# Rita-zi/WavTokenizer

Measured on AMD Instinct MI355X. Metric: audio-seconds/sec encode+decode, 24 kHz 3 s clips, higher is better.
Workload: dtype f32 (split-f16 x3 products)

## Files before the change

include/wavtokenizer_amd.h:

```cpp
#ifndef WAVTOKENIZER_AMD_H
#define WAVTOKENIZER_AMD_H

#include <stddef.h>
#include <stdint.h>

#ifdef __cplusplus
extern "C" {
#endif

typedef enum {
    WT_OK = 0,
    WT_ERR_INVALID = -1,
    WT_ERR_MISSING_TENSOR = -2,
    WT_ERR_SHAPE = -3,
    WT_ERR_HIP = -4,
    WT_ERR_NOT_INITED = -5,
    WT_ERR_RANGE = -6,
    WT_ERR_LSTM_SYNC = -7,
    WT_ERR_INDEX = -8
} wt_status;

enum wt_status_bits {
    WT_STATUS_BIT_LSTM = 1,
    WT_STATUS_BIT_RANGE = 2
// ... 140 lines not shown
    const float* B;
    const float* bias;
    const float* R;
    const float* gamma;
    float* C;
    float* C2;
    uint32_t* status;
} wt_gemm_desc;
typedef struct {
    int32_t BM, BN, waves_m, waves_n, stages, ks, prod, staged, bias_cache, G, tiles;
} wt_launch_form;
size_t wt_gemm_probe_workspace_bytes(const wt_gemm_desc* d);
int wt_gemm_probe(const wt_gemm_desc* d, wt_launch_form* form, void* workspace, void* stream);

enum { WT_OP_GN_APPLY = 0, WT_OP_GN_STATS = 1, WT_OP_ROWNORM = 2, WT_OP_SOFTMAX = 3, WT_OP_ISTFT_OLA = 4, WT_OP_CONV_FIRST = 5,
       WT_OP_CONV_LAST = 6, WT_OP_TRANSPOSE = 7, WT_OP_CONVTR = 8, WT_OP_ROW_SUMSQ = 9, WT_OP_S32_AMAX = 10 };
enum { WT_OPK_GN_TILE = 1, WT_OPK_GN_CHUNK = 2, WT_OPK_GN_STATS = 3, WT_OPK_ROWNORM = 4, WT_OPK_DWCONV_LN = 5,
       WT_OPK_SOFTMAX_REG = 6, WT_OPK_SOFTMAX_RMW = 7, WT_OPK_ISTFT_OLA = 8, WT_OPK_CONV_FIRST = 9, WT_OPK_CONV_LAST32 = 10,
       WT_OPK_CONV_LAST = 11, WT_OPK_TRANSPOSE = 12, WT_OPK_CONVTR = 13, WT_OPK_ROW_SUMSQ = 14, WT_OPK_S32_AMAX = 15 };
typedef struct {
    int32_t size;
    int32_t op;
    int32_t B, L, C;
    int32_t groups, mode, flag, out_s32;
    int32_t ld, k, stride, Cout, n_fft, hop, Kq;
    float eps;
    int64_t n;
    const void* x;
    const void *p0, *p1, *p2, *p3, *p4, *p5;
    void *y, *y2, *y3;
    uint32_t* status;
} wt_op_desc;
typedef struct {
    int32_t kernel;
    int32_t variant;
    int32_t variant2;
    int32_t grid_x, grid_y, grid_z, block, lds;
} wt_op_form;
int wt_op_probe(const wt_op_desc* d, wt_op_form* form, void* stream);

int wt_resblock(const float* x, const float* wav, const float* e0_w, const float* e0_b, const float* w3, const float* b3,
                const float* w1, const float* b1, const float* ws, const float* bs, float* y, int32_t B, int64_t T,
                int32_t C, int32_t elu_out, int32_t out_s32, int32_t fp32_chain, void* stream);
int wt_resblock_down(const float* wav, const float* e0_w, const float* e0_b, const float* w3, const float* b3, const float* w1,
                     const float* b1, const float* ws, const float* bs, const float* wd, const float* bd, float* y_down,
                     int32_t B, int64_t T, int32_t r, void* stream);

int wt_unit_run(const wt_plan* p, const float* x, float* y, void* workspace, void* stream);

int wt_model_take_bad_codes(const wt_model* m);


typedef struct wt_resampler wt_resampler;
int     wt_resampler_create(int32_t orig_sr, int32_t new_sr, int32_t device, wt_resampler** out);
void    wt_resampler_destroy(wt_resampler* r);
// ... 13 lines not shown
```

wavtokenizer_amd/_capi.py:

```python
from __future__ import annotations

import ctypes
import os
from ctypes import POINTER, c_char_p, c_float, c_int32, c_int64, c_size_t, c_void_p

_HERE = os.path.dirname(os.path.abspath(__file__))
LIB_PATH = os.environ.get("WAVTOK_HIP_LIB") or os.path.join(_HERE, "libwavtok_hip.so")

EXPORTS = [
    "wt_last_error", "wt_version", "wt_model_create", "wt_model_destroy", "wt_model_export_bytes", "wt_model_export", "wt_packed_info", "wt_packed_verify", "wt_packed_bytes",
    "wt_model_create_packed", "wt_model_hop", "wt_model_weight_bytes",
    "wt_plan_create", "wt_plan_create_ex", "wt_plan_range_sites", "wt_plan_range_report", "wt_model_persistent_lstm", "wt_device_info", "wt_plan_destroy", "wt_plan_workspace_bytes", "wt_plan_frames", "wt_plan_num_launches", "wt_plan_graph_replays",
    "wt_plan_find_buffer", "wt_plan_buffer_info", "wt_plan_buffer_name", "wt_plan_status", "wt_plan_num_steps", "wt_plan_step_name",
    "wt_plan_set_timing", "wt_plan_read_timing", "wt_model_split_ok", "wt_model_status", "wt_model_take_bad_codes", "wt_encode", "wt_codes_to_features",
    "wt_decode", "wt_seanet_decode", "wt_head", "wt_unit_run", "wt_sconv1d", "wt_linear", "wt_conv1d_s32", "wt_vq_workspace_bytes",
    "wt_vq_nearest", "wt_vq_nearest_f32", "wt_resblock", "wt_resblock_down", "wt_gemm_probe_workspace_bytes", "wt_gemm_probe", "wt_op_probe",
    "wt_resampler_create", "wt_resampler_destroy", "wt_resampler_out_length", "wt_convert_audio", "wt_pcm16",
    "wt_linear_overlap_add", "wt_encode_mixed", "wt_plan_min_clip_length", "wt_sconv_geometry",
]

WT_PLAN_ENCODE, WT_PLAN_DECODE, WT_PLAN_SEANET_DECODER, WT_PLAN_HEAD, WT_PLAN_UNIT_LSTM = 0, 1, 2, 3, 4
WT_PLAN_FLAG_KEEP_STAGES = 1
WT_PLAN_FLAG_FP32_GEMM = 2
WT_PLAN_FLAG_STEP_LSTM = 4
WT_PLAN_FLAG_GRAPH = 8
WT_PLAN_FLAG_UNFUSED = 16
WT_PLAN_FLAG_RANGE_REPORT = 32
WT_PLAN_FLAG_MIXED_LENGTH = 64
WT_SITE_ENCODER, WT_SITE_BB_EMBED, WT_SITE_RES0, WT_SITE_RES1, WT_SITE_ATTN, WT_SITE_RES2, WT_SITE_RES3 = 0, 1, 2, 3, 4, 5, 6
WT_SITE_CNX0, WT_SITE_HEAD, WT_SITE_SEANET_DECODER = 7, 40, 41
WT_ERR_INVALID = -1
# ... 18 lines not shown
                 ("M", c_int32), ("N", c_int32), ("K", c_int32)]
                + [(n, c_int32) for n in ("T_in", "T_out", "Cin", "taps", "stride", "dil", "pad_left", "pad_mode", "Tp",
                                         "K1", "nz", "tap_pair", "head_kb")]
                + [("alpha", c_float)]
                + [(n, c_int64) for n in ("a_bstride", "a_rstride", "a2_bstride", "a2_rstride", "w_rstride", "c_rstride",
                                         "r_rstride", "zA", "zW", "zC")]
                + [(n, c_void_p) for n in ("A", "A2", "B", "bias", "R", "gamma", "C", "C2", "status")])


class WtLaunchForm(ctypes.Structure):
    _fields_ = [(n, c_int32) for n in ("BM", "BN", "waves_m", "waves_n", "stages", "ks", "prod", "staged", "bias_cache", "G", "tiles")]


WT_OP_GN_APPLY, WT_OP_GN_STATS, WT_OP_ROWNORM, WT_OP_SOFTMAX, WT_OP_ISTFT_OLA, WT_OP_CONV_FIRST = 0, 1, 2, 3, 4, 5
WT_OP_CONV_LAST, WT_OP_TRANSPOSE, WT_OP_CONVTR, WT_OP_ROW_SUMSQ, WT_OP_S32_AMAX = 6, 7, 8, 9, 10
WT_OPK_NAMES = {1: "gn_tile", 2: "gn_chunk", 3: "gn_stats", 4: "rownorm", 5: "dwconv_ln", 6: "softmax_reg", 7: "softmax_rmw",
                8: "istft_ola", 9: "conv_first", 10: "conv_last32", 11: "conv_last", 12: "transpose", 13: "convtr",
                14: "row_sumsq", 15: "s32_amax"}


class WtOpDesc(ctypes.Structure):
    _fields_ = ([(n, c_int32) for n in ("size", "op", "B", "L", "C", "groups", "mode", "flag", "out_s32", "ld", "k", "stride",
                                        "Cout", "n_fft", "hop", "Kq")]
                + [("eps", c_float), ("n", c_int64)]
                + [(n, c_void_p) for n in ("x", "p0", "p1", "p2", "p3", "p4", "p5", "y", "y2", "y3", "status")])


class WtOpForm(ctypes.Structure):
    _fields_ = [(n, c_int32) for n in ("kernel", "variant", "variant2", "grid_x", "grid_y", "grid_z", "block", "lds")]


class WavTokError(RuntimeError):
    def __init__(self, msg, status=0):
# ... 74 lines not shown
    lib.wt_sconv1d.argtypes = [c_void_p, c_void_p, c_void_p, c_void_p, c_int32, c_int64, c_int32, c_int32, c_int32,
                               c_int32, c_int32, c_int32, c_void_p]
    lib.wt_linear.argtypes = [c_void_p, c_void_p, c_void_p, c_void_p, c_int64, c_int32, c_int32, c_int32, c_void_p, c_void_p]
    lib.wt_conv1d_s32.argtypes = [c_void_p, c_void_p, c_void_p, c_void_p, c_int32, c_int64, c_int32, c_int32, c_int32,
                                  c_int32, c_int32, c_void_p, c_void_p]
    lib.wt_vq_workspace_bytes.argtypes = [c_int64, c_int32, c_int32]
    lib.wt_vq_workspace_bytes.restype = c_size_t
    lib.wt_vq_nearest.argtypes = [c_void_p, c_void_p, c_int64, c_int32, c_int32, c_void_p, c_void_p, c_void_p]
    lib.wt_vq_nearest_f32.argtypes = [c_void_p, c_void_p, c_int64, c_int32, c_int32, c_void_p, c_void_p, c_void_p]
    lib.wt_resblock.argtypes = [c_void_p] * 11 + [c_int32, c_int64, c_int32, c_int32, c_int32, c_int32, c_void_p]
    lib.wt_resblock_down.argtypes = [c_void_p] * 12 + [c_int32, c_int64, c_int32, c_void_p]
    lib.wt_gemm_probe_workspace_bytes.argtypes = [POINTER(WtGemmDesc)]
    lib.wt_gemm_probe_workspace_bytes.restype = c_size_t
    lib.wt_gemm_probe.argtypes = [POINTER(WtGemmDesc), POINTER(WtLaunchForm), c_void_p, c_void_p]
    lib.wt_op_probe.argtypes = [POINTER(WtOpDesc), POINTER(WtOpForm), c_void_p]
    lib.wt_resampler_create.argtypes = [c_int32, c_int32, c_int32, POINTER(c_void_p)]
    lib.wt_resampler_destroy.argtypes = [c_void_p]
    lib.wt_resampler_destroy.restype = None
    lib.wt_resampler_out_length.argtypes = [c_void_p, c_int64]
    lib.wt_resampler_out_length.restype = c_int64
    lib.wt_convert_audio.argtypes = [c_void_p, c_void_p, c_int32, c_int32, c_int64, c_void_p, c_void_p]
    lib.wt_pcm16.argtypes = [c_void_p, c_int64, ctypes.c_float, c_int32, c_void_p, c_void_p, c_void_p]
    lib.wt_linear_overlap_add.argtypes = [c_void_p, c_void_p, c_int32, c_int64, c_int64, c_int64, c_int64, c_void_p, c_void_p]
    return lib


lib = _load()


def check(rc: int, what: str = "") -> None:
# ... 4 lines not shown
```

wavtokenizer_amd/csrc/capi.cpp:

```cpp
#include "model.h"

namespace wt {
static thread_local std::string g_err;
void set_error(const std::string& msg) { g_err = msg; }
thread_local LaunchCtx g_launch;
int device_cus() {
    static std::atomic<int> cache[64];
    int d = 0;
    (void)hipGetDevice(&d);
    d &= 63;
    int v = cache[d].load(std::memory_order_relaxed);
    if (v <= 0) {
        if (hipDeviceGetAttribute(&v, hipDeviceAttributeMultiprocessorCount, d) != hipSuccess || v <= 0) v = 256;
        cache[d].store(v, std::memory_order_relaxed);
    }
    return v;
}
}

using namespace wt;

static int alloc_host_words(wt_model* M, const char* who) {
    void* hp = nullptr;
    void* dp = nullptr;
// ... 728 lines not shown
            if (int rc = launch_fill_u32(scale_dev, bits, 16, s)) return rc;
            a.acc_scale = 1.f / scale;
        }
        if (int rc = launch_split_s32(d->B, ws + L.oB, L.nB, s, scale != 1.f ? scale_dev : nullptr)) return rc;
        if (int rc = launch_split_s32(d->A, ws, L.nA, s)) return rc;
        if (d->A2) if (int rc = launch_split_s32(d->A2, ws + L.oA2, L.nA2, s)) return rc;
        if (int rc = launch_gemm16s(a, d->epi, d->out, s)) return rc;
    }
    if (form) *form = wt_launch_form{lf.BM, lf.BN, lf.waves_m, lf.waves_n, lf.stages, lf.ks, lf.prod, lf.staged, lf.bias_cache, lf.G, lf.tiles};
    return WT_OK;
}

static int op_probe_check(const wt_op_desc* d) {
    auto bad = [](const char* m) { set_error(std::string("wt_op_probe: ") + m); return (int)WT_ERR_INVALID; };
    if (!d || d->size != (int32_t)sizeof(wt_op_desc)) return bad("descriptor missing or of another size");
    if (d->op < WT_OP_GN_APPLY || d->op > WT_OP_S32_AMAX) return bad("unknown op");
    auto al16 = [](const void* p) { return !(reinterpret_cast<uintptr_t>(p) & 15); };
    const void* ptrs[] = {d->p0, d->p1, d->p2, d->p3, d->p4, d->p5, d->y, d->y2, d->y3};
    for (const void* p : ptrs) if (!al16(p)) return bad("arrays must be 16-byte aligned");
    if (!d->x || (reinterpret_cast<uintptr_t>(d->x) & (d->op == WT_OP_SOFTMAX ? 3 : 15))) return bad("x missing or misaligned");
    if (reinterpret_cast<uintptr_t>(d->status) & 3) return bad("status misaligned");
    const bool shaped = d->op != WT_OP_SOFTMAX && d->op != WT_OP_ROW_SUMSQ && d->op != WT_OP_S32_AMAX;
    if (shaped && (d->B <= 0 || d->L <= 0)) return bad("extents must be positive");
    if (shaped && d->op != WT_OP_CONV_FIRST && d->op != WT_OP_ISTFT_OLA && (d->C <= 0 || (long)d->L * d->C >= (long)INT_MAX)) return bad("extents must be positive (and L * C < 2^31)");
    switch (d->op) {
    case WT_OP_GN_APPLY: case WT_OP_GN_STATS:
        if (!d->p0 || !d->p1 || !d->y2 || !d->y3 || (d->op == WT_OP_GN_APPLY && !d->y)) return bad("null argument");
        if (d->groups <= 0 || d->C % d->groups || d->C / d->groups > 256 || d->B > 65535) return bad("GroupNorm needs C % groups == 0, at most 256 channels per group, B <= 65535");
        break;
    case WT_OP_ROWNORM:
        if (!d->y || !d->p4 || !d->p5) return bad("null argument");
// ... 21 lines not shown
        if (!d->y) return bad("null argument");
        if (d->B > 65535 || (d->L + 31) / 32 > 65535) return bad("transpose: too many tiles for one launch");
        break;
    case WT_OP_CONVTR:
        if (!d->p0 || !d->p1 || !d->y) return bad("null argument");
        if (d->stride <= 0 || d->k < d->stride || d->Cout <= 0 || d->Cout % 4) return bad("convtr needs k >= stride > 0 and Cout % 4 == 0");
        break;
    case WT_OP_ROW_SUMSQ:
        if (!d->y) return bad("null argument");
        if (d->n <= 0 || d->C <= 0 || d->C % 4) return bad("row_sumsq needs rows > 0 and C % 4 == 0");
        break;
    case WT_OP_S32_AMAX:
        if (!d->y) return bad("null argument");
        if (d->n <= 0 || d->n % 32) return bad("s32_amax needs whole S32 groups of 32 values");
        break;
    }
    return WT_OK;
}

int wt_op_probe(const wt_op_desc* d, wt_op_form* form, void* stream) {
    if (int rc = op_probe_check(d)) return rc;
    hipStream_t s = static_cast<hipStream_t>(stream);
    auto F = [](const void* p) { return static_cast<const float*>(p); };
    auto W = [](void* p) { return static_cast<float*>(p); };
    OpForm lf;
    const LaunchCtx saved = g_launch;
    g_launch.status = reinterpret_cast<unsigned*>(d->status);
    g_launch.form = &lf;
    int rc = 0;
    switch (d->op) {
    case WT_OP_GN_APPLY:
        rc = launch_gn_apply(F(d->x), F(d->p0), F(d->p1), W(d->y2), W(d->y3), W(d->y), d->flag ? 1 : 0, d->B, d->L, d->C, d->groups, d->eps, s,
// ... 18 lines not shown
    case WT_OP_CONV_LAST:
        rc = launch_conv_last(F(d->x), F(d->p0), F(d->p1), W(d->y), d->B, d->L, d->C, d->k, d->flag ? 1 : 0, s);
        break;
    case WT_OP_TRANSPOSE:
        rc = launch_transpose(F(d->x), W(d->y), d->B, d->L, d->C, s, d->out_s32 ? 1 : 0);
        break;
    case WT_OP_CONVTR:
        rc = launch_convtr(F(d->x), F(d->p0), F(d->p1), W(d->y), d->B, d->L, d->C, d->Cout, d->k, d->stride, d->flag ? 1 : 0, s);
        break;
    case WT_OP_ROW_SUMSQ:
        rc = launch_row_sumsq(F(d->x), W(d->y), d->n, d->C, s);
        break;
    case WT_OP_S32_AMAX:
        rc = launch_s32_amax(d->x, d->n, static_cast<unsigned*>(d->y), s);
        break;
    }
    g_launch = saved;
    if (rc) return rc;
    if (form) *form = wt_op_form{lf.kernel, lf.variant, lf.variant2, (int32_t)lf.grid[0], (int32_t)lf.grid[1], (int32_t)lf.grid[2], (int32_t)lf.block, (int32_t)lf.lds};
    return WT_OK;
}

size_t wt_vq_workspace_bytes(int64_t N, int32_t D, int32_t bins) {
    const size_t np = std::max(gemm_vq_parts(bins), gemm16s_vq_parts(bins));
    return al256((size_t)N * D * 4) + al256((size_t)bins * D * 4) + al256((size_t)N * sizeof(float)) +
           2 * al256((size_t)N * np * sizeof(float)) + al256((size_t)bins * sizeof(float)) + 512;
}

static int vq_nearest(const float* x, const float* embed, int64_t N, int32_t D, int32_t bins, int64_t* codes_out,
                      void* workspace, void* stream, bool s32) {
// ... 69 lines not shown
```

wavtokenizer_amd/csrc/common.h:

```cpp
#pragma once
#include <hip/hip_runtime.h>
#include <stdint.h>
#include <stdio.h>
#include <stdlib.h>
#include <mutex>
#include <string>

namespace wt {

void set_error(const std::string& msg);

#define WT_HIP_CHECK(expr)                                                                      \
    do {                                                                                        \
        hipError_t _e = (expr);                                                                 \
        if (_e != hipSuccess) {                                                                 \
            ::wt::set_error(std::string(#expr) + ": " + hipGetErrorString(_e));                 \
            return -4;                                                                          \
        }                                                                                       \
    } while (0)

struct PerDeviceOnce {
    std::mutex mu;
    bool seen[64] = {};
    template <class F> int run(F&& f) {
        int d = 0;
        (void)hipGetDevice(&d);
        d &= 63;
        std::lock_guard<std::mutex> g(mu);
        if (seen[d]) return 0;
        if (int rc = f()) return rc;
        seen[d] = true;
        return 0;
    }
};

enum : unsigned { WT_STATUS_LSTM = 1u, WT_STATUS_RANGE = 2u };
enum OpKernel : int {
    OPK_NONE = 0, OPK_GN_TILE, OPK_GN_CHUNK, OPK_GN_STATS, OPK_ROWNORM, OPK_DWCONV_LN, OPK_SOFTMAX_REG, OPK_SOFTMAX_RMW,
    OPK_ISTFT_OLA, OPK_CONV_FIRST, OPK_CONV_LAST32, OPK_CONV_LAST, OPK_TRANSPOSE, OPK_CONVTR, OPK_ROW_SUMSQ, OPK_S32_AMAX
};
struct OpForm {
    int kernel = OPK_NONE;
    int variant = 0;
    int variant2 = 0;
    unsigned grid[3] = {0, 0, 0};
    unsigned block = 0;
    unsigned lds = 0;
};
struct LaunchCtx {
    unsigned* status = nullptr;
    OpForm* form = nullptr;
    unsigned long long* stamp_start = nullptr;
    unsigned long long* stamp_end = nullptr;
    bool stamp_used = false;
// ... 248 lines not shown
    int R;
};
struct ResblockMix {
    const int* T = nullptr;
    const int* Tread = nullptr;
};
bool resblock_fusable(int C);
int launch_resblock(const ResblockArgs& a, hipStream_t s);
int launch_resblock16(const ResblockArgs& a, hipStream_t s, const ResblockMix* mix = nullptr);
bool resblock16_down_fusable(int C, long T, int r, int k);
int launch_resblock16_down(const ResblockArgs& a, hipStream_t s, const ResblockMix* mix = nullptr);
int launch_mixed_geometry(const int* lengths, int* geom, int B, long Tpad, int tmin, int n_st, const int* kd, const int* rd,
                          int kf, hipStream_t s);
int launch_mixed_pad(const int* geom, int l_word, int64_t* codes, float* feat_ncl, float* emb_ncl, int B, int L, int D,
                     hipStream_t s);
int launch_convtr(const float* x, const float* w , const float* bias, float* y, int B, int Tin,
                  int Cin, int Cout, int k, int stride, int elu_in, hipStream_t s);

}
```

wavtokenizer_amd/csrc/model.h:

```cpp
#pragma once
#include "../../include/wavtokenizer_amd.h"
#include "common.h"

#include <algorithm>
#include <atomic>
#include <climits>
#include <cmath>
#include <cstring>
#include <functional>
#include <map>
#include <memory>
#include <mutex>
#include <string>
#include <vector>

namespace wt {

struct S32Copy {
    const void* p = nullptr;
    float acc_scale = 1.f;
    bool tap_pair = false;
};
struct ConvW {
    float* w = nullptr;
// ... 260 lines not shown

int build_model(wt_model* M, TensorMap& tm);
int build_splits(wt_model* M);
float s32_weight_scale(float amax);
size_t model_export_bytes(const wt_model* M);
int model_export(const wt_model* M, void* buf, size_t n);
int model_import(wt_model* M, const void* buf, size_t n);
int packed_info(const void* buf, size_t n, wt_arch* arch, int32_t* version, uint64_t* arch_hash);
int ensure_f32_weights(const wt_model* M);
size_t packed_bytes(const void* buf, size_t n);
int packed_verify(const void* buf, size_t n);
GemmArgs sconv_args(const ConvW& w, int B, long T, int stride, int dil);
GemmArgs zconv_args(const ConvW& w, int B, int L);
GemmArgs linear_args(const float* W, const float* bias, long M, int N, int K);
GemmArgs linear_args(const GemmW& W, const float* bias, long M, int N, int K);
int build_encode(wt_plan* P);
int build_decode(wt_plan* P);
int build_head(wt_plan* P);
int build_seanet_decoder(wt_plan* P);
int build_unit_lstm(wt_plan* P);
void plan_begin(wt_plan* P);
void plan_end(wt_plan* P);
inline long wave_samples(const wt_model* M, long L) {
    return M->arch.padding_same ? L * (long)M->arch.hop_length : (L - 1) * (long)M->arch.hop_length;
}

}
```

wavtokenizer_amd/csrc/plan.cpp:

```cpp
#include "model.h"

namespace wt {

static bool site_fp32(const wt_plan* P, int site) { return (P->fp32_sites >> site) & 1u; }
static bool plan_fp32(const wt_plan* P) {
    if ((P->flags & WT_PLAN_FLAG_FP32_GEMM) || !P->model->s32_ok) return true;
    if (P->kind == WT_PLAN_SEANET_DECODER) return !P->model->sd_s32_ok || site_fp32(P, SITE_SEADEC);
    if (P->kind == WT_PLAN_ENCODE || P->kind == WT_PLAN_UNIT_LSTM) return site_fp32(P, SITE_ENC);
    if (P->kind == WT_PLAN_HEAD) return site_fp32(P, SITE_HEAD);
    return false;
}
static bool plan_unfused(const wt_plan* P) { return P->flags & WT_PLAN_FLAG_UNFUSED; }
static bool plan_s32(const wt_plan* P) { return !plan_unfused(P) && !plan_fp32(P); }

static int gemm_auto(const wt_plan* P, const GemmArgs& a, int pro, int epi, hipStream_t s) {
    if (P->model->f32_stale.load()) if (int rc = ensure_f32_weights(P->model)) return rc;
    return launch_gemm(a, pro, epi, s);
}

static void set_s32(GemmArgs& a, const S32Copy& c) {
    a.W_hi = c.p; a.acc_scale = c.acc_scale; a.tap_pair = c.tap_pair ? 1 : 0;
}

static int gemm_s32(const GemmArgs& a, int epi, int out, hipStream_t s, const int* mix = nullptr) {
// ... 154 lines not shown
    });
    const int o = P->buf(name, (size_t)B * T * C, BUF_S32 | BUF_ELU);
    GemmArgs ac = sconv_args(sc, B, T, 1, 1);
    ac.W = cat.w; ac.w_rstride = cat.cin; ac.bias = cat.b; ac.K = cat.cin; ac.Cin = cat.cin;
    set_s32(ac, cat.s32);
    ac.K1 = C; ac.a2_bstride = T * (C / 2); ac.a2_rstride = C / 2;
    P->step({geom, x_raw, h, o}, [=](const RunCtx& c) {
        GemmArgs a = ac; a.A = P->ptr(c, x_raw) + x_off; a.A2 = P->ptr(c, h); a.C = P->ptr(c, o);
        if (x_bstride) a.a_bstride = x_bstride;
        const int* mix = geom >= 0 ? reinterpret_cast<const int*>(P->ptr(c, geom)) + mix_word + GEOM_SC : nullptr;
        return gemm_s32(a, EPI_BIAS_ELU, OUT_S32, c.stream, mix);
    });
    return o;
}

int build_encode(wt_plan* P) {
    const wt_model* M = P->model;
    const int B = P->B;
    const long T = P->T;
    const bool fold_e0 = !plan_unfused(P) && !M->stages.empty() && M->stages[0].C == 32 &&
                         M->e0_k == 7 && resblock_fusable(32);
    int x = -1;
    if (!fold_e0) {
        x = P->buf("enc.0", (size_t)B * T * M->e0_c);
        const int x0 = x;
        P->step({x0}, [=](const RunCtx& c) {
            return launch_conv_first(c.in_f, M->e0_w, M->e0_b, P->ptr(c, x0), B, T, M->e0_k, M->e0_c, c.stream);
        });
    }
    const bool fuse_elu = !plan_unfused(P);
    const bool s32 = plan_s32(P);
    struct Route { bool fused, down, s32; };
    std::vector<Route> route(M->stages.size());
    for (size_t si = 0; si < route.size(); ++si) {
        const ResStage& st = M->stages[si];
        Route& r = route[si];
        r.fused = resblock_fusable(st.C) && !plan_unfused(P);
        r.s32 = s32 && st.C % 32 == 0 && st.down.s32.p &&
                (r.fused || (si > 0 && route[si - 1].s32 && st.c3.s32.p && st.c1.s32.p && st.sc.s32.p));
        r.down = si == 0 && fold_e0 && r.fused && r.s32 && route.size() > 1 && resblock_fusable(M->stages[1].C) &&
                 st.down.cin == 32 && st.down.cout == 64 && resblock16_down_fusable(st.C, T, st.r, st.down.k);
    }
    const bool lstm_s32 = !route.empty() && route.back().s32 && M->enc_lstm.Wih0.s32.p;
    const bool tail_s32 = lstm_s32 && M->enc_final.s32.p && M->embed.s32.p;
    const bool mixed = P->flags & WT_PLAN_FLAG_MIXED_LENGTH;
    const int n_st = (int)route.size();
    int geom = -1;
    if (mixed) {
        bool ok = s32 && !(P->flags & (WT_PLAN_FLAG_KEEP_STAGES | WT_PLAN_FLAG_RANGE_REPORT)) && tail_s32 &&
                  n_st >= 2 && n_st <= GEOM_MAX_STAGES && route[0].down;
        for (int si = 1; si < n_st && ok; ++si)
            ok = route[si].s32 && (route[si].fused ? M->stages[si].C == 64 : M->stages[si].cat.s32.p != nullptr);
        for (const ResStage& st : M->stages) ok = ok && st.c3.k == 3 && st.sc.k == 1;
        if (!ok) {
// ... 33 lines not shown
                if (geom >= 0) { mix.T = mix_ptr(c, GEOM_T); mix.Tread = mix_ptr(c, GEOM_TREAD); }
                a.wav = c.in_f; a.e0_w = M->e0_w; a.e0_b = M->e0_b;
                a.W3 = st.c3.w; a.b3 = st.c3.b; a.W1 = st.c1.w; a.b1 = st.c1.b; a.Ws = st.sc.w; a.bs = st.sc.b;
                a.Wd = st.down.w; a.bd = st.down.b; a.y_down = P->ptr(c, y); a.R = st.r;
                a.B = B; a.T = (int)Tc; a.C = st.C;
                return launch_resblock16_down(a, c.stream, geom >= 0 ? &mix : nullptr);
            }, 1, "resblock.fused_down");
            x = y; Tc = ad.T_out; idx += 3;
            continue;
        }
        const std::string name = "enc." + std::to_string(idx);
        const int stage_word = GEOM_STAGE0 + (int)si * GEOM_STAGE_WORDS;
        if (r.fused)
            x = plan_resblock(P, st.c3, st.c1, st.sc, B, Tc, x, name, fuse_elu, (si == 0 && fold_e0) ? M : nullptr, 0, 0, r.s32,
                              mixed ? stage_word + GEOM_C3 : -1);
        else if (r.s32)
            x = plan_resblock_s32(P, st.c3, st.sc, st.cat, B, Tc, x, x_elu, name, 0, 0, mixed ? stage_word : -1);
        else
            x = plan_resblock(P, st.c3, st.c1, st.sc, B, Tc, x, name, fuse_elu);
        if (x < 0) return WT_ERR_INVALID;
        const bool next_s32 = !last && !route[si + 1].fused && route[si + 1].s32;
        const int y = P->buf(out, ynum, next_s32 ? BUF_S32 : BUF_F32);
        const int y2 = (next_s32 || (last && lstm_s32)) ? P->buf(out + ".s32", ynum, BUF_S32 | (next_s32 ? BUF_ELU : 0)) : -1;
        const int xin = x;
        P->step({geom, xin, y, y2}, [=](const RunCtx& c) {
            GemmArgs a = ad; a.A = P->ptr(c, xin); a.C = P->ptr(c, y);
            if (y2 >= 0) a.C2 = P->ptr(c, y2);
            return dense(P, r.s32, a, fuse_elu ? PRO_NONE : PRO_ELU, EPI_BIAS,
                         next_s32 ? OUT_S32_DUAL_ELU : (y2 >= 0 ? OUT_F32_AND_S32 : OUT_F32), c.stream,
                         geom >= 0 ? mix_ptr(c, stage_word + GEOM_DOWN) : nullptr);
        });
        if (next_s32) x_elu = y2;
        if (last) x_s32 = y2;
        x = y; Tc = ad.T_out; idx += 3;
    }
    const int L = (int)Tc;
// ... 378 lines not shown
```

Measured before the change: 37670.

## Fuse wide encoder resblocks (C=128/256) into one split-f16 MFMA kernel

Adds a fused kernel for encoder resblock stages with 128 or 256 channels. It splits the input into f16 hi/lo halves with and without ELU in LDS, runs the k=3 conv and the concatenated 1x1 conv with split-f16 MFMA, and keeps the intermediate h in LDS instead of round-tripping through global memory. The plan routes eligible non-mixed-length S32 stages to this kernel, replacing the two-GEMM S32 pair path. The cost is heavy LDS and register use, which limits occupancy to one workgroup per CU.

```diff
diff --git a/include/wavtokenizer_amd.h b/include/wavtokenizer_amd.h
--- a/include/wavtokenizer_amd.h
+++ b/include/wavtokenizer_amd.h
@@ -178,10 +178,12 @@
 int wt_gemm_probe(const wt_gemm_desc* d, wt_launch_form* form, void* workspace, void* stream);
 
 enum { WT_OP_GN_APPLY = 0, WT_OP_GN_STATS = 1, WT_OP_ROWNORM = 2, WT_OP_SOFTMAX = 3, WT_OP_ISTFT_OLA = 4, WT_OP_CONV_FIRST = 5,
-       WT_OP_CONV_LAST = 6, WT_OP_TRANSPOSE = 7, WT_OP_CONVTR = 8, WT_OP_ROW_SUMSQ = 9, WT_OP_S32_AMAX = 10 };
+       WT_OP_CONV_LAST = 6, WT_OP_TRANSPOSE = 7, WT_OP_CONVTR = 8, WT_OP_ROW_SUMSQ = 9, WT_OP_S32_AMAX = 10,
+       WT_OP_WIDE_RESBLOCK = 16  };
 enum { WT_OPK_GN_TILE = 1, WT_OPK_GN_CHUNK = 2, WT_OPK_GN_STATS = 3, WT_OPK_ROWNORM = 4, WT_OPK_DWCONV_LN = 5,
        WT_OPK_SOFTMAX_REG = 6, WT_OPK_SOFTMAX_RMW = 7, WT_OPK_ISTFT_OLA = 8, WT_OPK_CONV_FIRST = 9, WT_OPK_CONV_LAST32 = 10,
-       WT_OPK_CONV_LAST = 11, WT_OPK_TRANSPOSE = 12, WT_OPK_CONVTR = 13, WT_OPK_ROW_SUMSQ = 14, WT_OPK_S32_AMAX = 15 };
+       WT_OPK_CONV_LAST = 11, WT_OPK_TRANSPOSE = 12, WT_OPK_CONVTR = 13, WT_OPK_ROW_SUMSQ = 14, WT_OPK_S32_AMAX = 15,
+       WT_OPK_WIDE_RESBLOCK = 16 };
 typedef struct {
     int32_t size;
     int32_t op;
@@ -203,6 +205,9 @@
 } wt_op_form;
 int wt_op_probe(const wt_op_desc* d, wt_op_form* form, void* stream);
 
+enum { WT_ROUTE_FUSED = 0, WT_ROUTE_S32_PAIR = 1, WT_ROUTE_WIDE = 2, WT_ROUTE_F32 = 3 };
+int wt_encode_stage_route(int32_t C, int32_t plan_flags, int32_t s32_operands);
+
 int wt_resblock(const float* x, const float* wav, const float* e0_w, const float* e0_b, const float* w3, const float* b3,
                 const float* w1, const float* b1, const float* ws, const float* bs, float* y, int32_t B, int64_t T,
                 int32_t C, int32_t elu_out, int32_t out_s32, int32_t fp32_chain, void* stream);
diff --git a/wavtokenizer_amd/_capi.py b/wavtokenizer_amd/_capi.py
--- a/wavtokenizer_amd/_capi.py
+++ b/wavtokenizer_amd/_capi.py
@@ -14,7 +14,7 @@
     "wt_plan_find_buffer", "wt_plan_buffer_info", "wt_plan_buffer_name", "wt_plan_status", "wt_plan_num_steps", "wt_plan_step_name",
     "wt_plan_set_timing", "wt_plan_read_timing", "wt_model_split_ok", "wt_model_status", "wt_model_take_bad_codes", "wt_encode", "wt_codes_to_features",
     "wt_decode", "wt_seanet_decode", "wt_head", "wt_unit_run", "wt_sconv1d", "wt_linear", "wt_conv1d_s32", "wt_vq_workspace_bytes",
-    "wt_vq_nearest", "wt_vq_nearest_f32", "wt_resblock", "wt_resblock_down", "wt_gemm_probe_workspace_bytes", "wt_gemm_probe", "wt_op_probe",
+    "wt_vq_nearest", "wt_vq_nearest_f32", "wt_resblock", "wt_resblock_down", "wt_gemm_probe_workspace_bytes", "wt_gemm_probe", "wt_op_probe", "wt_encode_stage_route",
     "wt_resampler_create", "wt_resampler_destroy", "wt_resampler_out_length", "wt_convert_audio", "wt_pcm16",
     "wt_linear_overlap_add", "wt_encode_mixed", "wt_plan_min_clip_length", "wt_sconv_geometry",
 ]
@@ -63,9 +63,11 @@
 
 WT_OP_GN_APPLY, WT_OP_GN_STATS, WT_OP_ROWNORM, WT_OP_SOFTMAX, WT_OP_ISTFT_OLA, WT_OP_CONV_FIRST = 0, 1, 2, 3, 4, 5
 WT_OP_CONV_LAST, WT_OP_TRANSPOSE, WT_OP_CONVTR, WT_OP_ROW_SUMSQ, WT_OP_S32_AMAX = 6, 7, 8, 9, 10
+WT_OP_WIDE_RESBLOCK = 16
+WT_ROUTE_FUSED, WT_ROUTE_S32_PAIR, WT_ROUTE_WIDE, WT_ROUTE_F32 = 0, 1, 2, 3
 WT_OPK_NAMES = {1: "gn_tile", 2: "gn_chunk", 3: "gn_stats", 4: "rownorm", 5: "dwconv_ln", 6: "softmax_reg", 7: "softmax_rmw",
                 8: "istft_ola", 9: "conv_first", 10: "conv_last32", 11: "conv_last", 12: "transpose", 13: "convtr",
-                14: "row_sumsq", 15: "s32_amax"}
+                14: "row_sumsq", 15: "s32_amax", 16: "wide_resblock"}
 
 
 class WtOpDesc(ctypes.Structure):
@@ -170,6 +172,7 @@
     lib.wt_gemm_probe_workspace_bytes.restype = c_size_t
     lib.wt_gemm_probe.argtypes = [POINTER(WtGemmDesc), POINTER(WtLaunchForm), c_void_p, c_void_p]
     lib.wt_op_probe.argtypes = [POINTER(WtOpDesc), POINTER(WtOpForm), c_void_p]
+    lib.wt_encode_stage_route.argtypes = [c_int32, c_int32, c_int32]
     lib.wt_resampler_create.argtypes = [c_int32, c_int32, c_int32, POINTER(c_void_p)]
     lib.wt_resampler_destroy.argtypes = [c_void_p]
     lib.wt_resampler_destroy.restype = None
diff --git a/wavtokenizer_amd/csrc/capi.cpp b/wavtokenizer_amd/csrc/capi.cpp
--- a/wavtokenizer_amd/csrc/capi.cpp
+++ b/wavtokenizer_amd/csrc/capi.cpp
@@ -766,7 +766,7 @@
 static int op_probe_check(const wt_op_desc* d) {
     auto bad = [](const char* m) { set_error(std::string("wt_op_probe: ") + m); return (int)WT_ERR_INVALID; };
     if (!d || d->size != (int32_t)sizeof(wt_op_desc)) return bad("descriptor missing or of another size");
-    if (d->op < WT_OP_GN_APPLY || d->op > WT_OP_S32_AMAX) return bad("unknown op");
+    if ((d->op < WT_OP_GN_APPLY || d->op > WT_OP_S32_AMAX) && d->op != WT_OP_WIDE_RESBLOCK) return bad("unknown op");
     auto al16 = [](const void* p) { return !(reinterpret_cast<uintptr_t>(p) & 15); };
     const void* ptrs[] = {d->p0, d->p1, d->p2, d->p3, d->p4, d->p5, d->y, d->y2, d->y3};
     for (const void* p : ptrs) if (!al16(p)) return bad("arrays must be 16-byte aligned");
@@ -818,8 +818,35 @@
         if (!d->y) return bad("null argument");
         if (d->n <= 0 || d->n % 32) return bad("s32_amax needs whole S32 groups of 32 values");
         break;
-    }
-    return WT_OK;
+    case WT_OP_WIDE_RESBLOCK:
+        if (!d->p0 || !d->p1 || !d->p2 || !d->p3 || !d->p4 || !d->y) return bad("null argument");
+        if (!wide_resblock_fusable(d->C) || d->B > 65535 || (long)d->L * d->C >= 0x20000000L) return bad("wide_resblock needs C = 128 or 256, B <= 65535 and L * C < 2^29");
+        if ((reinterpret_cast<uintptr_t>(d->p4) & 255) || (reinterpret_cast<uintptr_t>(d->y) & 127)) return bad("wide_resblock needs a 256-byte aligned workspace and a 128-byte aligned y");
+        if (d->flag && (!d->p5 || (reinterpret_cast<uintptr_t>(d->p5) & 255))) return bad("the two-launch form needs a second, 256-byte aligned workspace");
+        break;
+    }
+    return WT_OK;
+}
+
+static int probe_split_weight(const float* w, long n, char* out, float* scale_dev, float* acc_scale, hipStream_t s) {
+    std::vector<float> h((size_t)n);
+    WT_HIP_CHECK(hipMemcpyAsync(h.data(), w, (size_t)n * 4, hipMemcpyDeviceToHost, s));
+    WT_HIP_CHECK(hipStreamSynchronize(s));
+    float amax = 0.f;
+    for (float v : h) {
+        if (!(std::fabs(v) <= 3.0e38f)) { set_error("wt_op_probe: a non-finite weight has no S32 copy"); return WT_ERR_INVALID; }
+        amax = std::max(amax, std::fabs(v));
+    }
+    const float scale = s32_weight_scale(amax);
+    uint32_t bits;
+    memcpy(&bits, &scale, 4);
+    if (int rc = launch_fill_u32(scale_dev, bits, 16, s)) return rc;
+    *acc_scale = 1.f / scale;
+    return launch_split_s32(w, out, n, s, scale != 1.f ? scale_dev : nullptr);
+}
+
+int wt_encode_stage_route(int32_t C, int32_t plan_flags, int32_t s32_operands) {
+    return encode_stage_route(C, plan_flags, s32_operands != 0);
 }
 
 int wt_op_probe(const wt_op_desc* d, wt_op_form* form, void* stream) {
@@ -868,6 +895,38 @@
     case WT_OP_S32_AMAX:
         rc = launch_s32_amax(d->x, d->n, static_cast<unsigned*>(d->y), s);
         break;
+    case WT_OP_WIDE_RESBLOCK: {
+        const long n3 = (long)(d->C / 2) * 3 * d->C, nc = (long)d->C * (d->C + d->C / 2);
+        char* ws = static_cast<char*>(const_cast<void*>(d->p4));
+        float* scales = reinterpret_cast<float*>(ws + (n3 + nc) * 4);
+        WideResblockArgs a;
+        a.x = F(d->x); a.b3 = F(d->p1); a.bc = F(d->p3); a.y = W(d->y); a.B = d->B; a.T = d->L; a.C = d->C;
+        a.W3 = ws; a.Wc = ws + n3 * 4;
+        rc = probe_split_weight(F(d->p0), n3, ws, scales, &a.acc_scale3, s);
+        if (!rc) rc = probe_split_weight(F(d->p2), nc, ws + n3 * 4, scales + 64, &a.acc_scalec, s);
+        if (!rc && !d->flag) rc = launch_wide_resblock(a, s);
+        if (!rc && d->flag) {
+            const int C = d->C, B = d->B, T = d->L;
+            const size_t nx = (size_t)B * T * C;
+            float* xs = static_cast<float*>(const_cast<void*>(d->p5));
+            float *xe = xs + nx, *h = xe + nx;
+            ConvW c3, cat;
+            c3.w = const_cast<float*>(F(d->p0)); c3.b = const_cast<float*>(a.b3); c3.cout = C / 2; c3.cin = C; c3.k = 3;
+            cat.w = const_cast<float*>(F(d->p2)); cat.b = const_cast<float*>(a.bc); cat.cout = C; cat.cin = C + C / 2; cat.k = 1;
+            rc = launch_wide_split(a.x, xs, xe, (long)nx, s);
+            GemmArgs a3 = sconv_args(c3, B, T, 1, 1);
+            a3.W_hi = a.W3; a3.acc_scale = a.acc_scale3; a3.A = xe; a3.C = h;
+            if (!rc) rc = launch_gemm16s(a3, EPI_BIAS_ELU, OUT_S32, s);
+            ConvW sc1 = cat; sc1.cin = C;
+            GemmArgs ac = sconv_args(sc1, B, T, 1, 1);
+            ac.W = cat.w; ac.w_rstride = cat.cin; ac.bias = cat.b; ac.K = cat.cin; ac.Cin = cat.cin;
+            ac.W_hi = a.Wc; ac.acc_scale = a.acc_scalec;
+            ac.K1 = C; ac.a2_bstride = (long)T * (C / 2); ac.a2_rstride = C / 2;
+            ac.A = xs; ac.A2 = h; ac.C = a.y;
+            if (!rc) rc = launch_gemm16s(ac, EPI_BIAS_ELU, OUT_S32, s);
+        }
+        break;
+    }
     }
     g_launch = saved;
     if (rc) return rc;
diff --git a/wavtokenizer_amd/csrc/common.h b/wavtokenizer_amd/csrc/common.h
--- a/wavtokenizer_amd/csrc/common.h
+++ b/wavtokenizer_amd/csrc/common.h
@@ -37,7 +37,8 @@
 enum : unsigned { WT_STATUS_LSTM = 1u, WT_STATUS_RANGE = 2u };
 enum OpKernel : int {
     OPK_NONE = 0, OPK_GN_TILE, OPK_GN_CHUNK, OPK_GN_STATS, OPK_ROWNORM, OPK_DWCONV_LN, OPK_SOFTMAX_REG, OPK_SOFTMAX_RMW,
-    OPK_ISTFT_OLA, OPK_CONV_FIRST, OPK_CONV_LAST32, OPK_CONV_LAST, OPK_TRANSPOSE, OPK_CONVTR, OPK_ROW_SUMSQ, OPK_S32_AMAX
+    OPK_ISTFT_OLA, OPK_CONV_FIRST, OPK_CONV_LAST32, OPK_CONV_LAST, OPK_TRANSPOSE, OPK_CONVTR, OPK_ROW_SUMSQ, OPK_S32_AMAX,
+    OPK_WIDE_RESBLOCK
 };
 struct OpForm {
     int kernel = OPK_NONE;
@@ -316,6 +317,22 @@
                           int kf, hipStream_t s);
 int launch_mixed_pad(const int* geom, int l_word, int64_t* codes, float* feat_ncl, float* emb_ncl, int B, int L, int D,
                      hipStream_t s);
+struct WideResblockArgs {
+    const float* x = nullptr;
+    long x_bstride = 0;
+    const void* W3 = nullptr;
+    const float* b3 = nullptr;
+    float acc_scale3 = 1.f;
+    const void* Wc = nullptr;
+    const float* bc = nullptr;
+    float acc_scalec = 1.f;
+    float* y = nullptr;
+    int B = 0, T = 0, C = 0;
+    unsigned* status = nullptr;
+};
+bool wide_resblock_fusable(int C);
+int launch_wide_resblock(const WideResblockArgs& a, hipStream_t s);
+int launch_wide_split(const float* x, float* xs, float* xe, long n, hipStream_t s);
 int launch_convtr(const float* x, const float* w , const float* bias, float* y, int B, int Tin,
                   int Cin, int Cout, int k, int stride, int elu_in, hipStream_t s);
 
diff --git a/wavtokenizer_amd/csrc/model.h b/wavtokenizer_amd/csrc/model.h
--- a/wavtokenizer_amd/csrc/model.h
+++ b/wavtokenizer_amd/csrc/model.h
@@ -298,6 +298,7 @@
 GemmArgs zconv_args(const ConvW& w, int B, int L);
 GemmArgs linear_args(const float* W, const float* bias, long M, int N, int K);
 GemmArgs linear_args(const GemmW& W, const float* bias, long M, int N, int K);
+int encode_stage_route(int C, int flags, bool s32_operands);
 int build_encode(wt_plan* P);
 int build_decode(wt_plan* P);
 int build_head(wt_plan* P);
diff --git a/wavtokenizer_amd/csrc/plan.cpp b/wavtokenizer_amd/csrc/plan.cpp
--- a/wavtokenizer_amd/csrc/plan.cpp
+++ b/wavtokenizer_amd/csrc/plan.cpp
@@ -192,6 +192,28 @@
     return o;
 }
 
+static int plan_resblock_wide(wt_plan* P, const ConvW& c3, const ConvW& cat, int B, long T, int xin, const std::string& name) {
+    const int C = cat.cout;
+    const int o = P->buf(name, (size_t)B * T * C, BUF_S32 | BUF_ELU);
+    P->step({xin, o}, [=](const RunCtx& c) {
+        WideResblockArgs a;
+        a.x = P->ptr(c, xin); a.y = P->ptr(c, o);
+        a.W3 = c3.s32.p; a.b3 = c3.b; a.acc_scale3 = c3.s32.acc_scale;
+        a.Wc = cat.s32.p; a.bc = cat.b; a.acc_scalec = cat.s32.acc_scale;
+        a.B = B; a.T = (int)T; a.C = C;
+        return launch_wide_resblock(a, c.stream);
+    });
+    return o;
+}
+
+int encode_stage_route(int C, int flags, bool s32_operands) {
+    if (flags & (WT_PLAN_FLAG_UNFUSED | WT_PLAN_FLAG_FP32_GEMM)) s32_operands = false;
+    if (resblock_fusable(C) && !(flags & WT_PLAN_FLAG_UNFUSED)) return WT_ROUTE_FUSED;
+    if (!s32_operands) return WT_ROUTE_F32;
+    if (wide_resblock_fusable(C) && !(flags & WT_PLAN_FLAG_MIXED_LENGTH)) return WT_ROUTE_WIDE;
+    return WT_ROUTE_S32_PAIR;
+}
+
 int build_encode(wt_plan* P) {
     const wt_model* M = P->model;
     const int B = P->B;
@@ -208,7 +230,7 @@
     }
     const bool fuse_elu = !plan_unfused(P);
     const bool s32 = plan_s32(P);
-    struct Route { bool fused, down, s32; };
+    struct Route { bool fused, down, s32, wide; };
     std::vector<Route> route(M->stages.size());
     for (size_t si = 0; si < route.size(); ++si) {
         const ResStage& st = M->stages[si];
@@ -216,6 +238,9 @@
         r.fused = resblock_fusable(st.C) && !plan_unfused(P);
         r.s32 = s32 && st.C % 32 == 0 && st.down.s32.p &&
                 (r.fused || (si > 0 && route[si - 1].s32 && st.c3.s32.p && st.c1.s32.p && st.sc.s32.p));
+        r.wide = encode_stage_route(st.C, P->flags, r.s32) == WT_ROUTE_WIDE && st.cat.s32.p && st.c3.k == 3 && st.sc.k == 1 &&
+                 st.c3.cin == st.C && st.c3.cout == st.C / 2 && st.cat.cout == st.C && st.cat.cin == st.C + st.C / 2 &&
+                 !st.c3.s32.tap_pair && !st.cat.s32.tap_pair;
         r.down = si == 0 && fold_e0 && r.fused && r.s32 && route.size() > 1 && resblock_fusable(M->stages[1].C) &&
                  st.down.cin == 32 && st.down.cout == 64 && resblock16_down_fusable(st.C, T, st.r, st.down.k);
     }
@@ -279,12 +304,14 @@
         if (r.fused)
             x = plan_resblock(P, st.c3, st.c1, st.sc, B, Tc, x, name, fuse_elu, (si == 0 && fold_e0) ? M : nullptr, 0, 0, r.s32,
                               mixed ? stage_word + GEOM_C3 : -1);
+        else if (r.wide)
+            x = plan_resblock_wide(P, st.c3, st.cat, B, Tc, x, name);
         else if (r.s32)
             x = plan_resblock_s32(P, st.c3, st.sc, st.cat, B, Tc, x, x_elu, name, 0, 0, mixed ? stage_word : -1);
         else
             x = plan_resblock(P, st.c3, st.c1, st.sc, B, Tc, x, name, fuse_elu);
         if (x < 0) return WT_ERR_INVALID;
-        const bool next_s32 = !last && !route[si + 1].fused && route[si + 1].s32;
+        const bool next_s32 = !last && !route[si + 1].fused && !route[si + 1].wide && route[si + 1].s32;
         const int y = P->buf(out, ynum, next_s32 ? BUF_S32 : BUF_F32);
         const int y2 = (next_s32 || (last && lstm_s32)) ? P->buf(out + ".s32", ynum, BUF_S32 | (next_s32 ? BUF_ELU : 0)) : -1;
         const int xin = x;
diff --git a/wavtokenizer_amd/csrc/wide_resblock.hip b/wavtokenizer_amd/csrc/wide_resblock.hip
--- /dev/null
+++ b/wavtokenizer_amd/csrc/wide_resblock.hip
@@ -0,0 +1,334 @@
+#include "common.h"
+
+namespace wt {
+
+typedef float f32x4 __attribute__((ext_vector_type(4)));
+typedef _Float16 f16x8 __attribute__((ext_vector_type(8)));
+typedef _Float16 f16x4 __attribute__((ext_vector_type(4)));
+
+namespace {
+
+__device__ __forceinline__ float elu_w(float x) { return elu_med3(x); }
+
+__device__ __forceinline__ void store_out16(float* dst, const f32x4 v) {
+    typedef unsigned u32x4_t __attribute__((ext_vector_type(4)));
+    const u32x4_t qv = __builtin_bit_cast(u32x4_t, v);
+    asm volatile("global_store_dwordx4 %0, %1, off sc1\n\ts_nop 1" :: "v"(dst), "v"(qv) : "memory");
+}
+
+template <int C, int BM, int WAVES_M>
+struct WideGeo {
+    static constexpr int NW = 8, NT = 64 * NW, WAVES_N = NW / WAVES_M;
+    static constexpr int WROWS = BM / WAVES_M;
+    static constexpr int NCH = C / 32;
+    static constexpr int RS = C * 4 + 128;
+    static constexpr int HS = C * 2 + 128;
+    static constexpr int XS_BYTES = BM * RS, XE_BYTES = (BM + 2) * RS;
+    static constexpr int LDS = XS_BYTES + XE_BYTES;
+    static constexpr int TM = WROWS / 16;
+    static constexpr int WN3 = C / 2 / WAVES_N, TN3 = WN3 / 16;
+    static constexpr int WNC = C / WAVES_N, TNC = WNC / 16;
+    static constexpr int NK3 = 3 * NCH, NKC = NCH + NCH / 2;
+    static_assert(WROWS % 16 == 0 && WN3 % 16 == 0 && WNC % 32 == 0, "16-row MFMA tiles, whole 32-column S32 groups per wave");
+    static_assert(BM * HS <= XE_BYTES && NW * 2048 <= XS_BYTES, "h aliases xe, the store scratch aliases xs");
+    static_assert(LDS <= 160 * 1024, "one workgroup per CU");
+};
+
+template <int C, int BM, int WAVES_M>
+__global__ __launch_bounds__(512, 2) void wide_resblock_kernel(const WideResblockArgs p) {
+    using G = WideGeo<C, BM, WAVES_M>;
+    constexpr int RS = G::RS, HS = G::HS, TM = G::TM, NCH = G::NCH;
+    extern __shared__ __attribute__((aligned(1024))) char smem_w[];
+    char* const xs = smem_w;
+    char* const xe = smem_w + G::XS_BYTES;
+    char* const hs = xe;
+
+    const int tid = threadIdx.x, lane = tid & 63;
+    const int wave = __builtin_amdgcn_readfirstlane(tid >> 6);
+    const int wave_m = wave / G::WAVES_N, wave_n = wave % G::WAVES_N, wrow0 = wave_m * G::WROWS;
+    const int r16 = lane & 15, q4 = lane >> 4;
+    const int b = blockIdx.y, t0 = blockIdx.x * BM;
+    const int T = p.T, Tp = T > 2 ? T : 2;
+    float amax = 0.f;
+
+    {
+        constexpr int UPR = C / 8, TOTAL = (BM + 2) * UPR, ITERS = (TOTAL + G::NT - 1) / G::NT;
+        const float* xb = p.x + (long)b * p.x_bstride;
+        f32x4 v[ITERS][2];
+#pragma unroll
+        for (int it = 0; it < ITERS; ++it) {
+            const int e = tid + it * G::NT;
+            const int j = e / UPR, u = e - j * UPR;
+            int pos = t0 - 1 + j;
+            pos = pos < 0 ? -pos : pos;
+            pos = pos >= Tp ? 2 * (Tp - 1) - pos : pos;
+            v[it][0] = v[it][1] = (f32x4){0.f, 0.f, 0.f, 0.f};
+            if (e < TOTAL && pos >= 0 && pos < T) {
+                const f32x4* src = reinterpret_cast<const f32x4*>(xb + (long)pos * C + u * 8);
+                v[it][0] = src[0];
+                v[it][1] = src[1];
+            }
+        }
+#pragma unroll
+        for (int it = 0; it < ITERS; ++it) {
+            const int e = tid + it * G::NT;
+            if (e >= TOTAL) continue;
+            const int j = e / UPR, u = e - j * UPR;
+            const int g = u >> 2, c = u & 3;
+            const f32x4 a0 = v[it][0], a1 = v[it][1];
+            f32x4 e0, e1;
+            e0.x = elu_w(a0.x); e0.y = elu_w(a0.y); e0.z = elu_w(a0.z); e0.w = elu_w(a0.w);
+            e1.x = elu_w(a1.x); e1.y = elu_w(a1.y); e1.z = elu_w(a1.z); e1.w = elu_w(a1.w);
+            amax = amax4(amax4(amax, a0.x, a0.y, a0.z, a0.w), a1.x, a1.y, a1.z, a1.w);
+            amax = amax4(amax4(amax, e0.x, e0.y, e0.z, e0.w), e1.x, e1.y, e1.z, e1.w);
+            f16x4 h0, l0, h1, l1;
+            split4_f16(e0.x, e0.y, e0.z, e0.w, h0, l0);
+            split4_f16(e1.x, e1.y, e1.z, e1.w, h1, l1);
+            {
+                const int sw = (j >> 1) & 7;
+                char* row = xe + j * RS + g * 128;
+                *reinterpret_cast<f16x8*>(row + ((c ^ sw) * 16)) = __builtin_shufflevector(h0, h1, 0, 1, 2, 3, 4, 5, 6, 7);
+                *reinterpret_cast<f16x8*>(row + (((4 + c) ^ sw) * 16)) = __builtin_shufflevector(l0, l1, 0, 1, 2, 3, 4, 5, 6, 7);
+            }
+            if (j >= 1 && j <= BM) {
+                split4_f16(a0.x, a0.y, a0.z, a0.w, h0, l0);
+                split4_f16(a1.x, a1.y, a1.z, a1.w, h1, l1);
+                const int r = j - 1, sw = (r >> 1) & 7;
+                char* row = xs + r * RS + g * 128;
+                *reinterpret_cast<f16x8*>(row + ((c ^ sw) * 16)) = __builtin_shufflevector(h0, h1, 0, 1, 2, 3, 4, 5, 6, 7);
+                *reinterpret_cast<f16x8*>(row + (((4 + c) ^ sw) * 16)) = __builtin_shufflevector(l0, l1, 0, 1, 2, 3, 4, 5, 6, 7);
+            }
+        }
+    }
+    __syncthreads();
+
+    auto read_a = [&](const char* base, int pitch, int row0, int g, f16x8& h, f16x8& l) {
+        const int row = row0 + r16, sw = (row >> 1) & 7;
+        const char* rp = base + row * pitch + g * 128;
+        h = *reinterpret_cast<const f16x8*>(rp + ((q4 ^ sw) * 16));
+        l = *reinterpret_cast<const f16x8*>(rp + (((4 + q4) ^ sw) * 16));
+    };
+    auto merge = [](const f32x4 m, const f32x4 c, float acc_s, float lo_s) {
+        f32x4 v;
+        v.x = fmaf(c.x, lo_s, m.x * acc_s);
+        v.y = fmaf(c.y, lo_s, m.y * acc_s);
+        v.z = fmaf(c.z, lo_s, m.z * acc_s);
+        v.w = fmaf(c.w, lo_s, m.w * acc_s);
+        return v;
+    };
+
+    {
+        constexpr int TN = G::TN3, NK = G::NK3, WD = 4;
+        const float acc_s = p.acc_scale3, lo_s = acc_s * (1.f / 2048.f);
+        const char* wrow[TN];
+#pragma unroll
+        for (int jn = 0; jn < TN; ++jn)
+            wrow[jn] = static_cast<const char*>(p.W3) + (long)(wave_n * G::WN3 + jn * 16 + r16) * (3 * C * 4) + q4 * 16;
+        f32x4 am[TM][TN], ac[TM][TN];
+#pragma unroll
+        for (int i = 0; i < TM; ++i)
+#pragma unroll
+            for (int jn = 0; jn < TN; ++jn) { am[i][jn] = (f32x4){0.f, 0.f, 0.f, 0.f}; ac[i][jn] = (f32x4){0.f, 0.f, 0.f, 0.f}; }
+        f16x8 wh[WD + 1][TN], wl[WD + 1][TN], ah[2][TM], al[2][TM];
+        auto load_w = [&](int k, int slot) {
+#pragma unroll
+            for (int jn = 0; jn < TN; ++jn) {
+                wh[slot][jn] = *reinterpret_cast<const f16x8*>(wrow[jn] + k * 128);
+                wl[slot][jn] = *reinterpret_cast<const f16x8*>(wrow[jn] + k * 128 + 64);
+            }
+        };
+        auto load_a = [&](int k, int slot) {
+            const int tap = k / NCH, g = k - tap * NCH;
+#pragma unroll
+            for (int i = 0; i < TM; ++i) read_a(xe, RS, wrow0 + i * 16 + tap, g, ah[slot][i], al[slot][i]);
+        };
+#pragma unroll
+        for (int k = 0; k < WD; ++k) load_w(k, k);
+        load_a(0, 0);
+#pragma unroll
+        for (int k = 0; k < NK; ++k) {
+            if (k + WD < NK) load_w(k + WD, (k + WD) % (WD + 1));
+            if (k + 1 < NK) load_a(k + 1, (k + 1) & 1);
+            __builtin_amdgcn_sched_barrier(0);
+#pragma unroll
+            for (int jn = 0; jn < TN; ++jn)
+#pragma unroll
+                for (int i = 0; i < TM; ++i) {
+                    am[i][jn] = __builtin_amdgcn_mfma_f32_16x16x32_f16(wh[k % (WD + 1)][jn], ah[k & 1][i], am[i][jn], 0, 0, 0);
+                    ac[i][jn] = __builtin_amdgcn_mfma_f32_16x16x32_f16(wl[k % (WD + 1)][jn], ah[k & 1][i], ac[i][jn], 0, 0, 0);
+                    ac[i][jn] = __builtin_amdgcn_mfma_f32_16x16x32_f16(wh[k % (WD + 1)][jn], al[k & 1][i], ac[i][jn], 0, 0, 0);
+                }
+            __builtin_amdgcn_sched_barrier(0);
+        }
+        f32x4 bq[TN];
+#pragma unroll
+        for (int jn = 0; jn < TN; ++jn) bq[jn] = *reinterpret_cast<const f32x4*>(p.b3 + wave_n * G::WN3 + jn * 16 + 4 * q4);
+        __syncthreads();
+#pragma unroll
+        for (int i = 0; i < TM; ++i)
+#pragma unroll
+            for (int jn = 0; jn < TN; ++jn) {
+                const f32x4 vb = merge(am[i][jn], ac[i][jn], acc_s, lo_s) + bq[jn];
+                f32x4 v;
+                v.x = elu_w(vb.x); v.y = elu_w(vb.y); v.z = elu_w(vb.z); v.w = elu_w(vb.w);
+                amax = amax4(amax, v.x, v.y, v.z, v.w);
+                f16x4 hi, lo;
+                split4_f16(v.x, v.y, v.z, v.w, hi, lo);
+                const int row = wrow0 + i * 16 + r16, sw = (row >> 1) & 7;
+                const int n = wave_n * G::WN3 + jn * 16 + 4 * q4;
+                char* rp = hs + row * HS + (n >> 5) * 128 + 2 * (n & 7);
+                *reinterpret_cast<f16x4*>(rp + ((((n & 31) >> 3) ^ sw) * 16)) = hi;
+                *reinterpret_cast<f16x4*>(rp + (((4 + ((n & 31) >> 3)) ^ sw) * 16)) = lo;
+            }
+    }
+    __syncthreads();
+
+    {
+        constexpr int TN = G::TNC, NK = G::NKC, WD = 3;
+        const float acc_s = p.acc_scalec, lo_s = acc_s * (1.f / 2048.f);
+        const char* wrow[TN];
+#pragma unroll
+        for (int jn = 0; jn < TN; ++jn)
+            wrow[jn] = static_cast<const char*>(p.Wc) + (long)(wave_n * G::WNC + jn * 16 + r16) * (NK * 128) + q4 * 16;
+        f32x4 am[TM][TN], ac[TM][TN];
+#pragma unroll
+        for (int i = 0; i < TM; ++i)
+#pragma unroll
+            for (int jn = 0; jn < TN; ++jn) { am[i][jn] = (f32x4){0.f, 0.f, 0.f, 0.f}; ac[i][jn] = (f32x4){0.f, 0.f, 0.f, 0.f}; }
+        f16x8 wh[WD + 1][TN], wl[WD + 1][TN], ah[2][TM], al[2][TM];
+        auto load_w = [&](int k, int slot) {
+#pragma unroll
+            for (int jn = 0; jn < TN; ++jn) {
+                wh[slot][jn] = *reinterpret_cast<const f16x8*>(wrow[jn] + k * 128);
+                wl[slot][jn] = *reinterpret_cast<const f16x8*>(wrow[jn] + k * 128 + 64);
+            }
+        };
+        auto load_a = [&](int k, int slot) {
+#pragma unroll
+            for (int i = 0; i < TM; ++i) {
+                if (k < NCH) read_a(xs, RS, wrow0 + i * 16, k, ah[slot][i], al[slot][i]);
+                else read_a(hs, HS, wrow0 + i * 16, k - NCH, ah[slot][i], al[slot][i]);
+            }
+        };
+#pragma unroll
+        for (int k = 0; k < WD; ++k) load_w(k, k);
+        load_a(0, 0);
+#pragma unroll
+        for (int k = 0; k < NK; ++k) {
+            if (k + WD < NK) load_w(k + WD, (k + WD) % (WD + 1));
+            if (k + 1 < NK) load_a(k + 1, (k + 1) & 1);
+            __builtin_amdgcn_sched_barrier(0);
+#pragma unroll
+            for (int jn = 0; jn < TN; ++jn)
+#pragma unroll
+                for (int i = 0; i < TM; ++i) {
+                    am[i][jn] = __builtin_amdgcn_mfma_f32_16x16x32_f16(wh[k % (WD + 1)][jn], ah[k & 1][i], am[i][jn], 0, 0, 0);
+                    ac[i][jn] = __builtin_amdgcn_mfma_f32_16x16x32_f16(wl[k % (WD + 1)][jn], ah[k & 1][i], ac[i][jn], 0, 0, 0);
+                    ac[i][jn] = __builtin_amdgcn_mfma_f32_16x16x32_f16(wh[k % (WD + 1)][jn], al[k & 1][i], ac[i][jn], 0, 0, 0);
+                }
+            __builtin_amdgcn_sched_barrier(0);
+        }
+        f32x4 bq[TN];
+#pragma unroll
+        for (int jn = 0; jn < TN; ++jn) bq[jn] = *reinterpret_cast<const f32x4*>(p.bc + wave_n * G::WNC + jn * 16 + 4 * q4);
+        __syncthreads();
+        char* sc = xs + wave * 2048;
+        float* yb = p.y + ((long)b * T + t0) * C;
+#pragma unroll
+        for (int i = 0; i < TM; ++i)
+#pragma unroll
+            for (int jg = 0; jg < TN / 2; ++jg) {
+#pragma unroll
+                for (int jh = 0; jh < 2; ++jh) {
+                    const int jn = 2 * jg + jh;
+                    const f32x4 vb = merge(am[i][jn], ac[i][jn], acc_s, lo_s) + bq[jn];
+                    f32x4 v;
+                    v.x = elu_w(vb.x); v.y = elu_w(vb.y); v.z = elu_w(vb.z); v.w = elu_w(vb.w);
+                    amax = amax4(amax, v.x, v.y, v.z, v.w);
+                    f16x4 hi, lo;
+                    split4_f16(v.x, v.y, v.z, v.w, hi, lo);
+                    const int cw = 16 * jh + 4 * q4, sww = (r16 >> 1) & 7;
+                    *reinterpret_cast<f16x4*>(sc + r16 * 128 + (((cw >> 3) ^ sww) * 16) + 2 * (cw & 7)) = hi;
+                    *reinterpret_cast<f16x4*>(sc + r16 * 128 + (((4 + (cw >> 3)) ^ sww) * 16) + 2 * (cw & 7)) = lo;
+                }
+                f32x4 q[2];
+#pragma unroll
+                for (int it = 0; it < 2; ++it) {
+                    const int r = 8 * it + (lane >> 3), ch = lane & 7;
+                    q[it] = *reinterpret_cast<const f32x4*>(sc + r * 128 + ((ch ^ ((r >> 1) & 7)) * 16));
+                }
+#pragma unroll
+                for (int it = 0; it < 2; ++it) {
+                    const int r = wrow0 + i * 16 + 8 * it + (lane >> 3), ch = lane & 7;
+                    if (t0 + r < T) store_out16(yb + (long)r * C + wave_n * G::WNC + jg * 32 + 4 * ch, q[it]);
+                }
+            }
+    }
+    range_report(p.status, amax);
+}
+
+template <int C, int BM, int WAVES_M>
+int launch_wide(const WideResblockArgs& a, hipStream_t s) {
+    using G = WideGeo<C, BM, WAVES_M>;
+    static PerDeviceOnce attr_once;
+    if (int rc = attr_once.run([&]() -> int {
+        WT_HIP_CHECK(hipFuncSetAttribute(reinterpret_cast<const void*>(wide_resblock_kernel<C, BM, WAVES_M>),
+                                         hipFuncAttributeMaxDynamicSharedMemorySize, G::LDS));
+        return 0;
+    })) return rc;
+    const dim3 grid((a.T + BM - 1) / BM, a.B);
+    if (g_launch.form) {
+        OpForm& f = *g_launch.form;
+        f.kernel = OPK_WIDE_RESBLOCK; f.variant = C; f.variant2 = BM;
+        f.grid[0] = grid.x; f.grid[1] = grid.y; f.grid[2] = 1; f.block = G::NT; f.lds = G::LDS;
+    }
+    hipLaunchKernelGGL((wide_resblock_kernel<C, BM, WAVES_M>), grid, dim3(G::NT), G::LDS, s, a);
+    WT_HIP_CHECK(hipGetLastError());
+    return 0;
+}
+
+__global__ __launch_bounds__(256) void wide_split_kernel(const float* __restrict__ x, float* __restrict__ xs, float* __restrict__ xe, long n4) {
+    for (long i = (long)blockIdx.x * blockDim.x + threadIdx.x; i < n4; i += (long)gridDim.x * blockDim.x) {
+        const f32x4 v = reinterpret_cast<const f32x4*>(x)[i];
+        f32x4 e;
+        e.x = elu_w(v.x); e.y = elu_w(v.y); e.z = elu_w(v.z); e.w = elu_w(v.w);
+        f16x4 hi, lo;
+        const long g = ((i * 4) >> 5) * 64 + ((i * 4) & 31);
+        split4_f16(v.x, v.y, v.z, v.w, hi, lo);
+        *reinterpret_cast<f16x4*>(reinterpret_cast<_Float16*>(xs) + g) = hi;
+        *reinterpret_cast<f16x4*>(reinterpret_cast<_Float16*>(xs) + g + 32) = lo;
+        split4_f16(e.x, e.y, e.z, e.w, hi, lo);
+        *reinterpret_cast<f16x4*>(reinterpret_cast<_Float16*>(xe) + g) = hi;
+        *reinterpret_cast<f16x4*>(reinterpret_cast<_Float16*>(xe) + g + 32) = lo;
+    }
+}
+
+}
+
+int launch_wide_split(const float* x, float* xs, float* xe, long n, hipStream_t s) {
+    if (n <= 0 || n % 32) { set_error("wide_split: element count must be a positive multiple of 32"); return -1; }
+    const long n4 = n / 4;
+    const int blocks = (int)((n4 + 255) / 256 < 8192 ? (n4 + 255) / 256 : 8192);
+    hipLaunchKernelGGL(wide_split_kernel, dim3(blocks), dim3(256), 0, s, x, xs, xe, n4);
+    WT_HIP_CHECK(hipGetLastError());
+    return 0;
+}
+
+bool wide_resblock_fusable(int C) { return C == 128 || C == 256; }
+
+int launch_wide_resblock(const WideResblockArgs& a_in, hipStream_t s) {
+    WideResblockArgs a = a_in;
+    if (!wide_resblock_fusable(a.C)) { set_error("wide_resblock: C must be 128 or 256"); return -1; }
+    if (!a.x || !a.W3 || !a.b3 || !a.Wc || !a.bc || !a.y) { set_error("wide_resblock: null argument"); return -1; }
+    if (a.B <= 0 || a.B > 65535 || a.T <= 0 || (long)a.T * a.C >= 0x20000000L) { set_error("wide_resblock: B in 1 .. 65535 and T * C < 2^29"); return -1; }
+    if (!a.x_bstride) a.x_bstride = (long)a.T * a.C;
+    if ((reinterpret_cast<uintptr_t>(a.x) & 15) || (a.x_bstride % 4) || (reinterpret_cast<uintptr_t>(a.W3) & 127) ||
+        (reinterpret_cast<uintptr_t>(a.Wc) & 127) || (reinterpret_cast<uintptr_t>(a.y) & 127) ||
+        (reinterpret_cast<uintptr_t>(a.b3) & 15) || (reinterpret_cast<uintptr_t>(a.bc) & 15)) {
+        set_error("wide_resblock: x and the biases must be 16-byte, the S32 arrays 128-byte aligned"); return -1;
+    }
+    if (!a.status) a.status = g_launch.status;
+    return a.C == 128 ? launch_wide<128, 96, 2>(a, s) : launch_wide<256, 64, 1>(a, s);
+}
+
+}
```

Result: no change. 37630 (median of 2 runs) (-0.1%).
